# robotics-upo/social_force_window_planner

Measured on AMD Instinct MI355X. Metric: scored trajectories/sec (v x w samples x steps) @ N pedestrians; cmd_vel match, higher is better.
Workload: dtype f64

## Files before the change

include/sfw_hip.h:

```cpp
#ifndef SFW_HIP_H_
#define SFW_HIP_H_

#include <stdint.h>

#ifdef __cplusplus
extern "C" {
#endif

#define SFW_ABI_VERSION 2

typedef enum sfw_status {
  SFW_OK = 0,
  SFW_ERR_INVALID_ARG = -1,
  SFW_ERR_NO_DEVICE = -2,
  SFW_ERR_HIP = -3,
  SFW_ERR_STATE = -4,
  SFW_ERR_UNSUPPORTED = -5
} sfw_status;

#define SFW_COST_INVALID (-1.0)
#define SFW_COST_SKIPPED (-2.0)

#define SFW_ROBOT_ID_NONE INT32_MIN

// ... 155 lines not shown
int sfw_plan_shared_prefix(const double *linvels, int32_t nv,
                           const double *angvels, int32_t nw, double vx0,
                           double vtheta0, double acc_x, double acc_theta,
                           double sim_time, int32_t num_steps,
                           int32_t n_agents, int32_t *level_ends,
                           int64_t *level_classes, int32_t cap,
                           int32_t *n_levels);
int sfw_plan_axis_classes(const double *targets, int32_t n, double v0, double a_max, double dt, int32_t max_p,
                          int32_t form, int32_t *counts, int32_t *classes, int32_t *n_levels, int32_t *closed_form);
int sfw_plan_row_blocks(const double *linvels, int32_t nv, const double *angvels, int32_t nw, double vx0,
                        double vtheta0, double acc_x, double acc_theta, double sim_time, int32_t num_steps,
                        int32_t n_agents, int32_t R, int32_t *row0);
#define SFW_K2_AUTO (-1)
#define SFW_K2_REGISTER 0
#define SFW_K2_FLAT 1
int sfw_set_k2_form(sfw_handle h, int32_t form);
int sfw_set_timing(sfw_handle h, int32_t enabled);
int sfw_last_launch_ms(sfw_handle h, int32_t which, float *ms_out);
int sfw_last_clock_ghz(sfw_handle h, double *ghz_out);
int sfw_grid_points(sfw_handle h, int64_t index, double *points_xyth,
                    int32_t points_cap, int32_t *n_points);
int sfw_grid_points_batch(sfw_handle h, int64_t first, int64_t count, double *points_xyth, int32_t *n_points);
int sfw_set_points_capture(sfw_handle h, int32_t enabled);
void *sfw_stream(sfw_handle h);

#define SFW_TERM_VEL 0
#define SFW_TERM_DISTANCE 1
#define SFW_TERM_ANGLE 2
#define SFW_TERM_COSTMAP 3
#define SFW_TERM_SOCIAL 4
#define SFW_N_TERMS 5
#define SFW_RESCORE_MAX_K 1024
typedef struct sfw_weights {
  double vel, distance, angle, costmap, social;
} sfw_weights;
int sfw_set_terms_capture(sfw_handle h, int32_t enabled);
int sfw_grid_rescore(sfw_handle h, const sfw_weights *w, int32_t K, sfw_best *best_out, double *costs_out);
int sfw_grid_terms(sfw_handle h, int64_t first, int64_t count, double *terms_out);

#define SFW_BLEND_MAX_L 16
typedef struct sfw_blend_stat {
  double lambda;
  double j_min;
  double eta;
  double sum_w2;
  int64_t n_valid;
// ... 135 lines not shown
```

social_force_window_planner_amd/_abi.py:

```python
import ctypes as C

SFW_OK = 0
SFW_ERR_INVALID_ARG = -1
SFW_ERR_NO_DEVICE = -2
SFW_ERR_HIP = -3
SFW_ERR_STATE = -4
SFW_ERR_UNSUPPORTED = -5

SFW_COST_INVALID = -1.0
SFW_COST_SKIPPED = -2.0

SFW_PRECISION_F64 = 0
SFW_PRECISION_F32 = 1
SFW_PRECISION_F64_STRICT = 2

SFW_K2_AUTO, SFW_K2_REGISTER, SFW_K2_FLAT = -1, 0, 1
SFW_ORG_NONE, SFW_ORG_REGISTER_1, SFW_ORG_REGISTER_2, SFW_ORG_FLAT = 0, 1, 2, 3


class SfwParams(C.Structure):
    _fields_ = [
        ("max_vel_x", C.c_double),
        ("sim_time", C.c_double),
        ("sim_granularity", C.c_double),
# ... 190 lines not shown
    "sfw_ensemble_aggregate",
    "sfw_ensemble_last_us",
    "sfw_samples_stage",
    "sfw_score_samples",
    "sfw_sequences_stage",
    "sfw_score_sequences",
    "sfw_score_one_crowd",
    "sfw_grid_crowd",
    "sfw_grid_blend",
    "sfw_sequences_perturb_stage",
    "sfw_score_perturbed",
    "sfw_sequences_knots",
    "sfw_sequences_normals",
    "sfw_ensemble_score_sequences",
    "sfw_ensemble_score_perturbed",
    "sfw_ensemble_blend",
    "sfw_sequences_control_cost",
    "sfw_grid_blend_control",
    "sfw_mppi_run",
    "sfw_ensemble_blend_control",
    "sfw_ensemble_mppi_run",
    "sfw_ensemble_set_risk",
    "sfw_ensemble_get_risk",
)
SFW_TERM_VEL, SFW_TERM_DISTANCE, SFW_TERM_ANGLE, SFW_TERM_COSTMAP, SFW_TERM_SOCIAL = 0, 1, 2, 3, 4
SFW_N_TERMS = 5
SFW_RESCORE_MAX_K = 1024


class SfwWeights(C.Structure):

    _fields_ = [("vel", C.c_double), ("distance", C.c_double), ("angle", C.c_double), ("costmap", C.c_double),
                ("social", C.c_double)]


SFW_BLEND_MAX_L = 16


class SfwBlendStat(C.Structure):

    _fields_ = [("lambda_", C.c_double), ("j_min", C.c_double), ("eta", C.c_double), ("sum_w2", C.c_double),
                ("n_valid", C.c_int64), ("index_min", C.c_int64)]

    def as_dict(self):
        d = {"lambda": self.lambda_, "j_min": self.j_min, "eta": self.eta, "sum_w2": self.sum_w2, "n_valid": self.n_valid,
             "index_min": self.index_min}
# ... 71 lines not shown
```

social_force_window_planner_amd/csrc/sfw_capi.hip:

```cpp

#include "sfw_device.h"

#include <dlfcn.h>
#include <link.h>

#include <algorithm>
#include <chrono>
#include <cmath>
#include <condition_variable>
#include <functional>
#include <mutex>
#include <thread>
#include <cstdio>
#include <cstdlib>
#include <cstring>
#include <limits>
#include <new>
#include <string>
#include <vector>

namespace {

template <typename T> struct dev_buf {
  T *p = nullptr;
  size_t cap = 0;
  dev_buf() = default;
  dev_buf(const dev_buf &) = delete;
  dev_buf &operator=(const dev_buf &) = delete;
  hipError_t reserve(size_t n) {
    if (n <= cap) return hipSuccess;
    if (p) (void)hipFree(p);
    p = nullptr;
    cap = 0;
    size_t want = n + n / 8 + 16;
    hipError_t e = hipMalloc(reinterpret_cast<void **>(&p), want * sizeof(T));
    if (e == hipSuccess) cap = want;
    return e;
  }
  void release() {
    if (p) (void)hipFree(p);
    p = nullptr;
    cap = 0;
  }
};

struct pinned_buf {
  char *p = nullptr;
  size_t cap = 0;
  hipEvent_t done = nullptr;
  bool pending = false;
  pinned_buf() = default;
  pinned_buf(const pinned_buf &) = delete;
  pinned_buf &operator=(const pinned_buf &) = delete;
  hipError_t wait() {
    if (!pending) return hipSuccess;
    pending = false;
    return hipEventSynchronize(done);
  }
  hipError_t reserve(size_t bytes) {
    hipError_t e = wait();
    if (e != hipSuccess) return e;
    if (!done && (e = hipEventCreateWithFlags(&done, hipEventDisableTiming)) != hipSuccess) return e;
    if (bytes <= cap) return hipSuccess;
    if (p) (void)hipHostFree(p);
    p = nullptr;
    cap = 0;
    const size_t want = bytes + bytes / 4 + 256;
    e = hipHostMalloc(reinterpret_cast<void **>(&p), want, hipHostMallocDefault);
// ... 53 lines not shown
  dev_buf<double> ctrl_bias, mppi_plan;
  pinned_buf pin_mppi;
  void release() {
    ctrl_bias.release();
    mppi_plan.release();
    pin_mppi.release();
  }
};

}

struct sfw_planner_s {
  struct config {
    int n_cu = SFW_DEFAULT_CUS, n_xcd = SFW_DEFAULT_CUS / SFW_CUS_PER_XCD;
    std::vector<int> prefix_env;
    bool pin_rest_on = true;
    long spin_us = 20000;
    bool arena_direct_on = true;
    size_t mirror_max_bytes = size_t(64) << 20;
    int obs_tasks_force = -1;
    size_t table_budget_bytes = size_t(8) << 30;
    bool owns_streams = true;
    bool batch_member = false;
  } cfg;

  struct switches {
    sfw_params params;
    uint64_t params_epoch = 1;
    int k2_form = SFW_K2_AUTO;
    bool timing = false;
    bool capture_points = false;
    bool capture_terms = false;
  } live;

  struct world_state {
    map_geometry map_new{0, 0, 0, 0, 0};
    bool have_costmap = false;
    bool cells_dirty = false;
    std::vector<double> footprint;
    int K = 0;
    agent_set agents;
  } world;

  struct stage_record {
    bool valid = false;
    std::vector<double> lin, ang;
    int nv = 0, nw = 0;
    sfw_robot_state rs{};
    sfw_goal_args ga{};
    double vy_samp = 0.0;
    int skip_zero = 1;
    int64_t index_base = 0;
    bool list = false;
    std::vector<double> vy;
    int nk = 1;
    std::vector<int32_t> knot_step;
    const int32_t *d_knot_step = nullptr;
    bool perturbed = false, zero_admitted = false, normals_kept = false;
    sfw_perturb_dev pert{};
    int K = 0, A = 0, O = 0, NG = 0, n_grp_mem = 0;
    bool person_pinned = false;
// ... 12 lines not shown
    std::vector<std::pair<int32_t, int32_t>> rest_pairs;
    std::vector<double> rest_pv;
    size_t pin_doubles = 0;
    std::vector<double> pin_pos;
    std::vector<sfw_agent_const> pin_cst;
    std::vector<int> prefix_steps;
    std::vector<chunk_plan> prefix_chunks;
    size_t prefix_o_col_cls = 0;
    int prefix_S = 0;
    int64_t prefix_chunk = 0;
    int64_t prefix_class_steps = 0, prefix_last_classes = 0;
    std::vector<int32_t> cls_ints;
    int64_t cls_max = 0;
    bool cls_two = false;
    const int32_t *d_cls_tab = nullptr;
    int64_t table_chunk = 0;
    uint64_t plan_epoch = 0;
    bool arena_pending = false;
    size_t arena_from = 0, arena_bytes = 0;
    bool early_poses = false;
    bool early_poses_timed = false;
    bool early_poses_terms = false;
    bool clock_cleared = false;
  } st;

  struct launch_record {
    bool launched = false;
    bool timed = false;
    bool cycle = false;
    bool fetched = false;
    bool mirrored = false;
    bool captured = false;
    int cap_S = 0;
    bool terms = false;
    int n_chunks = 1;
  } last;
  uint64_t launch_seq = 0;

  int device = 0;
  hipStream_t stream = nullptr;
  hipStream_t side = nullptr;
  hipEvent_t ev_poses = nullptr, ev_side = nullptr;
  sfw_split_streams split{nullptr, nullptr, nullptr};
  hipEvent_t ev[5] = {nullptr, nullptr, nullptr, nullptr, nullptr};
  std::vector<hipEvent_t> chunk_ev;
  std::string err;
  const void *shared_cols = nullptr;

  dev_buf<uint8_t> cells;
  dev_buf<char> arena;
  dev_buf<uint16_t> pair_tab;
  int pair_tab_A = -1;
  dev_buf<unsigned> cycle_counter;
  dev_buf<int32_t> d_cls, cls_dead[2];
  dev_buf<sfw_cls_agent> cls_state[2];
  dev_buf<int32_t> status, coll_step;
  dev_buf<double> base_cost, costs;
  dev_buf<sfw_unit> ptab, cs_tab;
  dev_buf<int16_t> fcode;
  dev_buf<sfw_sel> partials;
  dev_buf<double> points;
  dev_buf<int32_t> n_points;
  dev_buf<unsigned long long> clock;
  dev_buf<char> one_out;
  dev_buf<int32_t> pts_status, pts_coll;
  dev_buf<double> pts_base, pts_costs;
  dev_buf<sfw_unit> pts_ptab, pts_cs;
  dev_buf<int16_t> pts_fcode;
  pinned_buf pin_map, pin_arena, pin_out, pin_cls;
  pinned_buf pin_one;
  pinned_buf pin_mirror;
  pinned_buf pin_cap;
  dev_buf<double> terms;
  dev_buf<sfw_weights> rescore_w;
  dev_buf<sfw_sel> rescore_partials;
  dev_buf<double> rescore_costs;
  pinned_buf pin_rescore;
  blend_buffers blend;
  mppi_buffers mppi;
  dev_buf<double> normals;
  pinned_buf pin_knots;
  dev_buf<char> crowd_out;
// ... 106 lines not shown
  L.rs = h->st.rs;
  L.ga = h->st.ga;
  L.vy_samp = h->st.vy_samp;
  L.skip_zero_sample = h->st.skip_zero;
  L.linvels = h->st.d_linvels;
  L.angvels = h->st.d_angvels;
  L.nv = h->st.nv;
  L.nw = h->st.nw;
  L.vy_samps = h->st.d_vy;
  L.list = h->st.list ? 1 : 0;
  L.n_knots = h->st.nk;
  L.knot_step = h->st.d_knot_step;
  L.knot_stride = h->st.nv;
  L.chunk_begin = begin;
  L.chunk_count = count;
  L.cells = h->st.d_cells;
  L.size_x = h->st.map.size_x;
  L.size_y = h->st.map.size_y;
  L.origin_x = h->st.map.origin_x;
  L.origin_y = h->st.map.origin_y;
  L.resolution = h->st.map.resolution;
  L.footprint = h->st.d_footprint;
  L.K = h->st.K;
  L.agent_pos = h->st.d_agent_pos;
  L.agent_vel = h->st.d_agent_vel;
  L.agent_c = h->st.d_agent_c;
  L.agent_rest = h->st.d_agent_rest;
  L.pin_rest = h->st.d_pin_rest;
  L.A = h->st.A;
  L.obstacles = h->st.d_obstacles;
  L.O = h->st.O;
  L.agent_grp = h->st.d_agent_grp;
  L.grp_off = h->st.d_grp_off;
  L.grp_mem = h->st.d_grp_mem;
  L.NG = h->st.NG;
  L.n_grp_mem = h->st.n_grp_mem;
  L.n_cu = h->cfg.n_cu;
  L.n_xcd = h->cfg.n_xcd;
  sfw_derive(L);
  if (h->cfg.obs_tasks_force >= 0 && L.O > 0) L.k.obs_tasks = h->cfg.obs_tasks_force;
  L.pair_tab = h->pair_tab.p;
  L.status = h->status.p;
  L.base_cost = h->base_cost.p;
  L.costs = h->costs.p;
  L.coll_step = h->coll_step.p;
  L.ptab = h->ptab.p;
// ... 668 lines not shown
  return {stage_request::LIST, vx, vy, vtheta, n, 1, 1, nullptr, nullptr, 0.0, 0, index_base};
}
stage_request sequences_request(const double *vx, const double *vy, const double *vtheta, int32_t n, int32_t K,
                                const int32_t *knot_step, int64_t index_base) {
  return {stage_request::SEQUENCES, vx, vy, vtheta, n, 1, K, knot_step, nullptr, 0.0, 0, index_base};
}
stage_request perturbed_request(const perturb_source *dev, int32_t n, int32_t K, const int32_t *knot_step, int64_t index_base) {
  return {stage_request::PERTURBED, nullptr, nullptr, nullptr, n, 1, K, knot_step, dev, 0.0, 0, index_base};
}

const char *stage_null_refusal(const sfw_robot_state *rs, const sfw_goal_args *args, const stage_request &q) {
  if (!rs || (!q.drawn() && (!q.lin || !q.ang)) || !args || q.nv <= 0 || q.nw <= 0) return "null pointer or non-positive sample count";
  return nullptr;
}
const char *stage_finite_refusal(const sfw_robot_state *rs, const sfw_goal_args *args, const stage_request &q) {
  if (!all_finite(&rs->x, 6) || !all_finite(&args->acc_x, 5) || !std::isfinite(q.vy_samp))
    return "non-finite robot state, goal argument or sample velocity";
  const size_t rows = q.kn() * static_cast<size_t>(q.nv);
  if (!q.drawn() && (!all_finite(q.lin, rows) || !all_finite(q.ang, q.kn() * q.n_ang()) || (q.vy_list && !all_finite(q.vy_list, rows))))
    return "non-finite sample velocity";
  return nullptr;
}

int stage_common(sfw_handle h, const sfw_robot_state *rs, const sfw_goal_args *args, const stage_request &q) {
  if (!h) return SFW_ERR_INVALID_ARG;
  const std::string what = q.name();
  const auto [kind, lin, vy_list, ang, nv, nw, nk, knot_step, dev, vy_samp, skip_zero, index_base] = q;
  const size_t kn = q.kn(), n_ang = q.n_ang();
  const bool has_vy = dev ? dev->vy : vy_list != nullptr;
  if (const char *why = stage_null_refusal(rs, args, q)) return fail(h, SFW_ERR_INVALID_ARG, what + ": " + why);
  if (!h->world.have_costmap) return fail(h, SFW_ERR_STATE, what + ": no costmap set (sfw_set_costmap)");
  if (const char *why = stage_finite_refusal(rs, args, q)) return fail(h, SFW_ERR_INVALID_ARG, what + ": " + why);
  drop_stage(h);
  host_phases ph("stage:");
  SFW_HIP(h, hipSetDevice(h->device));
  const agent_set &ag = h->world.agents;
  const map_geometry &map = h->world.map_new;
  const size_t n_cells = static_cast<size_t>(map.size_x) * map.size_y;
  const bool merge = n_cells <= kMapMergeMax;
  if (h->world.cells_dirty && !merge) {
    SFW_HIP(h, h->cells.reserve(n_cells));
    SFW_HIP(h, hipMemcpyAsync(h->cells.p, h->pin_map.p, n_cells, hipMemcpyHostToDevice, h->stream));
    SFW_HIP(h, h->pin_map.mark(h->stream));
    h->world.cells_dirty = false;
  }
  ph.mark("check+setdev");
  h->st.perturbed = dev != nullptr;
  h->st.zero_admitted = dev && dev->zero_admitted;
  if (dev) h->st.pert = dev->args;
  h->st.normals_kept = false;
  if (dev) {
    h->st.lin.clear();
    h->st.ang.clear();
  } else {
    h->st.lin.assign(lin, lin + kn * nv);
    h->st.ang.assign(ang, ang + kn * n_ang);
  }
  h->st.list = q.is_list();
  if (vy_list) h->st.vy.assign(vy_list, vy_list + kn * nv);
  else h->st.vy.clear();
  h->st.nk = static_cast<int>(kn);
  if (knot_step) h->st.knot_step.assign(knot_step, knot_step + kn);
  else h->st.knot_step.clear();
  h->st.K = h->world.K;
  h->st.A = ag.A;
  h->st.O = ag.O;
  h->st.NG = ag.NG;
  h->st.n_grp_mem = ag.n_grp_mem;
  h->st.person_pinned = ag.person_pinned;
  h->st.nv = nv;
  h->st.nw = nw;
  h->st.rs = *rs;
  h->st.ga = *args;
  h->st.vy_samp = vy_samp;
  h->st.skip_zero = skip_zero;
  h->st.index_base = index_base;
  h->st.map = map;
  int plan_err = SFW_OK;
  const int64_t chunk = plan_tables_host(h, &plan_err);
  if (plan_err) return plan_err;
  ph.mark("plan");
  auto up16 = [](size_t b) { return (b + 15) & ~size_t(15); };
  const size_t cells_head = merge ? up16(n_cells) : 0;
  {
    const bool rest = !ag.rest_pairs.empty();
    const size_t o_fp = cells_head, o_ag = o_fp + up16(sizeof(double) * (h->world.footprint.empty() ? 2 : h->world.footprint.size())),
                 o_lin = o_ag + up16(ag.blob.size()), o_ang = o_lin + up16(sizeof(double) * kn * nv),
// ... 82 lines not shown
  const int64_t T = static_cast<int64_t>(nv) * nw;
  SFW_HIP(h, h->status.reserve(T));
  SFW_HIP(h, h->coll_step.reserve(T));
  SFW_HIP(h, h->base_cost.reserve(T));
  SFW_HIP(h, h->costs.reserve(T + (sizeof(sfw_sel) + sizeof(double) - 1) / sizeof(double)));
  h->st.d_sel = reinterpret_cast<sfw_sel *>(h->costs.p + T);
  SFW_HIP(h, h->partials.reserve(sfw_argmin_partials(T)));
  ph.mark("reserve");
  if (dev) {
    double *z = nullptr;
    if (dev->keep_normals) {
      SFW_HIP(h, h->normals.reserve(3 * kn * static_cast<size_t>(nv)));
      z = h->normals.p;
    }
    SFW_HIP(h, sfw_launch_perturb(dev->args, nv, static_cast<int>(kn), index_base, const_cast<double *>(h->st.d_linvels),
                                  const_cast<double *>(h->st.d_vy), const_cast<double *>(h->st.d_angvels), z, h->stream));
    h->st.normals_kept = dev->keep_normals;
    ph.mark("perturb");
  }
  if (int e = plan_tables_device(h, chunk, true)) return e;
  if (T > 1024)
    if (int e = flush_arena(h)) return e;
  ph.mark("tables+K1a");
  if (merge) {
    h->world.cells_dirty = false;
    h->st.cells_in_arena = true;
    h->st.arena_cells_bytes = cells_head;
  }
  h->st.valid = true;
  return SFW_OK;
}

int flush_arena(sfw_handle h) {
  if (!h->st.arena_pending) return SFW_OK;
  h->st.arena_pending = false;
  hipError_t e = hipMemcpyAsync(h->arena.p + h->st.arena_from, h->pin_arena.p + h->st.arena_from, h->st.arena_bytes,
                                hipMemcpyHostToDevice, h->stream);
  if (e == hipSuccess) e = h->pin_arena.mark(h->stream);
  if (e != hipSuccess) {
    drop_stage(h);
    return hip_fail(h, e, "flush_arena: arena copy");
  }
  return SFW_OK;
}

struct launch_prep {
// ... 591 lines not shown
  if (hipGetDeviceCount(&count) != hipSuccess || count <= 0) return SFW_ERR_NO_DEVICE;
  if (device < 0 || device >= count) return SFW_ERR_INVALID_ARG;
  sfw_handle h = new (std::nothrow) sfw_planner_s();
  if (!h) return SFW_ERR_HIP;
  h->live.params = *params;
  h->device = device;
  if (const char *b = std::getenv("SFW_PREFIX")) {
    for (const char *q = b; *q;) {
      char *end = nullptr;
      const long v = std::strtol(q, &end, 10);
      if (end == q) break;
      if (v >= 0) h->cfg.prefix_env.push_back(static_cast<int>(v));
      q = (*end == ',') ? end + 1 : end;
    }
    std::sort(h->cfg.prefix_env.begin(), h->cfg.prefix_env.end());
    h->cfg.prefix_env.erase(std::unique(h->cfg.prefix_env.begin(), h->cfg.prefix_env.end()), h->cfg.prefix_env.end());
  }
  if (const char *b = std::getenv("SFW_FORCE_FLAT")) h->live.k2_form = std::atoi(b) == 1 ? SFW_K2_FLAT : std::atoi(b) == 0 ? SFW_K2_REGISTER : SFW_K2_AUTO;
  if (const char *b = std::getenv("SFW_PIN_REST")) h->cfg.pin_rest_on = std::atoi(b) != 0;
  if (const char *b = std::getenv("SFW_SPIN_US")) h->cfg.spin_us = std::max(0L, std::atol(b));
  if (const char *b = std::getenv("SFW_ARENA_DIRECT")) h->cfg.arena_direct_on = std::atoi(b) != 0;
  if (const char *b = std::getenv("SFW_MIRROR_MAX_MB")) h->cfg.mirror_max_bytes = static_cast<size_t>(std::max(0L, std::atol(b))) << 20;
  if (const char *b = std::getenv("SFW_OBS_TASKS")) h->cfg.obs_tasks_force = std::atoi(b) != 0 ? 1 : 0;
  if (const char *b = std::getenv("SFW_TABLE_BUDGET_MB")) {
    long mb = std::atol(b);
    if (mb > 0) h->cfg.table_budget_bytes = static_cast<size_t>(mb) << 20;
  }
  hipError_t e = hipSetDevice(device);
  if (e == hipSuccess) {
    hipDeviceProp_t prop;
    if (hipGetDeviceProperties(&prop, device) == hipSuccess && prop.multiProcessorCount > 0) h->cfg.n_cu = prop.multiProcessorCount;
    h->cfg.n_cu = env_device_cus(h->cfg.n_cu);
    int xccs = 0;
    if (!std::getenv("SFW_DEVICE_CUS") && hipDeviceGetAttribute(&xccs, hipDeviceAttributeNumberOfXccs, device) == hipSuccess && xccs >= 1)
      h->cfg.n_xcd = xccs;
    else
      h->cfg.n_xcd = std::max(1, h->cfg.n_cu / SFW_CUS_PER_XCD);
    (void)hipGetLastError();
    if (const char *b = std::getenv("SFW_DEVICE_XCDS")) {
      const long v = std::atol(b);
      if (v >= 1 && v <= 64) h->cfg.n_xcd = static_cast<int>(v);
    }
  }
  if (stream) {
    h->cfg.owns_streams = false;
    h->stream = stream;
// ... 15 lines not shown
    return SFW_ERR_HIP;
  }
  *out = h;
  return SFW_OK;
}

int destroy_handle(sfw_handle h) {
  (void)hipSetDevice(h->device);
  if (h->stream) (void)hipStreamSynchronize(h->stream);
  if (h->side) (void)hipStreamSynchronize(h->side);
  h->cells.release();
  h->arena.release();
  h->pair_tab.release();
  h->crowd_pair_tab.release();
  h->crowd_out.release();
  h->pin_crowd.release();
  h->status.release();
  h->coll_step.release();
  h->base_cost.release();
  h->costs.release();
  h->ptab.release();
  h->cs_tab.release();
  h->fcode.release();
  h->partials.release();
  h->clock.release();
  h->cycle_counter.release();
  h->pin_cap.release();
  h->terms.release();
  h->rescore_w.release();
  h->rescore_partials.release();
  h->rescore_costs.release();
  h->pin_rescore.release();
  h->blend.release();
  h->mppi.release();
  h->normals.release();
  h->pin_knots.release();
  h->points.release();
  h->n_points.release();
  h->one_out.release();
  h->pts_status.release();
  h->pts_coll.release();
  h->pts_base.release();
  h->pts_costs.release();
  h->pts_ptab.release();
  h->pts_cs.release();
  h->pts_fcode.release();
// ... 44 lines not shown
}

const char *sfw_last_error(sfw_handle h) { return h ? h->err.c_str() : "null handle"; }

int sfw_set_costmap(sfw_handle h, const uint8_t *cells, uint32_t size_x, uint32_t size_y, double origin_x,
                    double origin_y, double resolution) {
  if (!h) return SFW_ERR_INVALID_ARG;
  if (!cells || size_x == 0 || size_y == 0 || !(resolution > 0))
    return fail(h, SFW_ERR_INVALID_ARG, "set_costmap: null cells, zero size or non-positive resolution");
  if (!std::isfinite(origin_x) || !std::isfinite(origin_y) || !std::isfinite(resolution))
    return fail(h, SFW_ERR_INVALID_ARG, "set_costmap: origin or resolution is not finite");
  if (size_x > SFW_MAX_MAP_AXIS_CELLS || size_y > SFW_MAX_MAP_AXIS_CELLS || static_cast<uint64_t>(size_x) * size_y > SFW_MAX_MAP_CELLS)
    return fail(h, SFW_ERR_INVALID_ARG, "set_costmap: more than SFW_MAX_MAP_AXIS_CELLS cells on an axis or SFW_MAX_MAP_CELLS in all");
  SFW_HIP(h, hipSetDevice(h->device));
  const size_t n = static_cast<size_t>(size_x) * size_y;
  if (h->world.have_costmap && h->pin_map.p && n <= h->pin_map.cap && h->world.map_new.size_x == size_x && h->world.map_new.size_y == size_y &&
      h->world.map_new.origin_x == origin_x && h->world.map_new.origin_y == origin_y && h->world.map_new.resolution == resolution &&
      std::memcmp(h->pin_map.p, cells, n) == 0)
    return SFW_OK;
  SFW_HIP(h, h->pin_map.reserve(n));
  std::memcpy(h->pin_map.p, cells, n);
  h->world.map_new = {size_x, size_y, origin_x, origin_y, resolution};
  h->world.cells_dirty = true;
  h->world.have_costmap = true;
  return SFW_OK;
}

int sfw_set_footprint(sfw_handle h, const double *xy, int32_t K) {
  if (!h) return SFW_ERR_INVALID_ARG;
  if (K < 0 || (K > 0 && !xy)) return fail(h, SFW_ERR_INVALID_ARG, "set_footprint: bad arguments");
  h->world.footprint.assign(xy, xy + 2 * static_cast<size_t>(K));
  h->world.K = K;
  return SFW_OK;
}

int sfw_set_agents(sfw_handle h, const sfw_agent *agents, int32_t A, const double *obstacles_xy, int32_t O) {
  if (!h) return SFW_ERR_INVALID_ARG;
  if (A < 0 || O < 0 || (A > 0 && !agents) || (O > 0 && !obstacles_xy))
    return fail(h, SFW_ERR_INVALID_ARG, "set_agents: bad arguments");
  for (int i = 0; i < A; ++i) {
    const sfw_agent &a = agents[i];
    if (!all_finite(&a.x, 4) || !std::isfinite(a.desired_velocity) || !std::isfinite(a.radius) ||
        (a.has_goal && !(all_finite(&a.goal_x, 2) && std::isfinite(a.goal_radius))))
      return fail(h, SFW_ERR_INVALID_ARG, "set_agents: non-finite field in agent " + std::to_string(i));
  }
  if (O > 0 && !all_finite(obstacles_xy, 2 * static_cast<size_t>(O)))
// ... 362 lines not shown
      float ms = 0.0f;
      const int a = 3 * c + (which == 1 ? 0 : 1);
      SFW_HIP(h, hipEventElapsedTime(&ms, h->chunk_ev[a], h->chunk_ev[a + 1]));
      total += ms;
    }
    *ms_out = total;
    return SFW_OK;
  }
  int a = 0, b = 3;
  switch (which) {
    case 0: a = 0; b = 3; break;
    case 1: a = 0; b = 1; break;
    case 2: a = 1; b = 2; break;
    case 3: a = 2; b = 3; break;
    default: return fail(h, SFW_ERR_INVALID_ARG, "last_launch_ms: which must be 0..3");
  }
  SFW_HIP(h, hipEventElapsedTime(ms_out, h->ev[a], h->ev[b]));
  return SFW_OK;
}

int sfw_set_points_capture(sfw_handle h, int32_t enabled) {
  if (!h) return SFW_ERR_INVALID_ARG;
  h->live.capture_points = enabled != 0;
  return SFW_OK;
}

int sfw_set_terms_capture(sfw_handle h, int32_t enabled) {
  if (!h) return SFW_ERR_INVALID_ARG;
  h->live.capture_terms = enabled != 0;
  if (!h->live.capture_terms) {
    h->last.terms = false;
    h->st.early_poses_terms = false;
    if (h->terms.p) {
      SFW_HIP(h, hipSetDevice(h->device));
      SFW_HIP(h, hipStreamSynchronize(h->stream));
      h->terms.release();
    }
  }
  return SFW_OK;
}

int sfw_grid_rescore(sfw_handle h, const sfw_weights *w, int32_t K, sfw_best *best_out, double *costs_out) {
  if (!h) return SFW_ERR_INVALID_ARG;
  if (!w || !best_out) return fail(h, SFW_ERR_INVALID_ARG, "grid_rescore: weights or best_out is NULL");
  if (K < 1 || K > SFW_RESCORE_MAX_K) return fail(h, SFW_ERR_INVALID_ARG, "grid_rescore: K out of [1, SFW_RESCORE_MAX_K]");
  if (!all_finite(reinterpret_cast<const double *>(w), static_cast<size_t>(K) * SFW_N_TERMS))
// ... 1614 lines not shown
```

social_force_window_planner_amd/csrc/sfw_device.h:

```cpp
#ifndef SFW_DEVICE_H_
#define SFW_DEVICE_H_

#include <hip/hip_runtime.h>
#include <stdint.h>

#include "../../include/sfw_hip.h"


#define SFW_DEFAULT_CUS 256
#define SFW_CUS_PER_XCD 32

enum : int32_t { SFW_ST_VALID = 0, SFW_ST_INVALID = 1, SFW_ST_SKIPPED = 2 };

struct __attribute__((aligned(32))) sfw_robot_step {
  double x, y, vx, vy;
};

struct __attribute__((aligned(32))) sfw_pose_frame {
  double x, y, c, s;
};

struct __attribute__((aligned(16))) sfw_unit {
  double a, b;
};
// ... 100 lines not shown
  sfw_unit *ptab;
  sfw_unit *cs_tab;
  int64_t row_units;
  int16_t *fcode;
  int64_t rstep_stride;
  double *points;
  int32_t *n_points;
  unsigned long long *clock_probe;
  int64_t index_base;
  unsigned *cycle_counter;
  sfw_sel *sel_out;
  double *costs_host;
  sfw_sel *sel_host;
  const char *arena_host;
  char *arena_dev;
  uint32_t arena_bytes;
  double *terms;
  int64_t terms_T;
  const double *vy_samps;
  int32_t list;
  int32_t n_knots;
  const int32_t *knot_step;
  int64_t knot_stride;
};

__device__ __forceinline__ void sfw_put_term(double *terms, int64_t T, int64_t t, int k, double v) {
  if (terms) terms[k * T + t] = v;
}
__device__ __forceinline__ void sfw_put_terms3(double *terms, int64_t T, int64_t t, double vel, double d, double ang) {
  if (!terms) return;
  terms[SFW_TERM_VEL * T + t] = vel;
  terms[SFW_TERM_DISTANCE * T + t] = d;
  terms[SFW_TERM_ANGLE * T + t] = ang;
}
__device__ __forceinline__ void sfw_put_terms_sentinel(double *terms, int64_t T, int64_t t, double sentinel) {
  if (!terms) return;
  for (int k = 0; k < SFW_N_TERMS; ++k) terms[k * T + t] = sentinel;
}


struct sfw_crowd_out {
  double *state;
  double *work;
  int32_t *has_goal;
};

void sfw_derive(sfw_launch &L);

hipError_t sfw_launch_rollout(const sfw_launch &L, hipStream_t stream);
hipError_t sfw_launch_rollout_poses(const sfw_launch &L, hipStream_t stream);
hipError_t sfw_launch_rollout_costmap(const sfw_launch &L, hipStream_t stream);
struct sfw_split_streams {
  hipStream_t side;
  hipEvent_t fork, join;
};
hipError_t sfw_launch_social(const sfw_launch &L, hipStream_t stream, const sfw_split_streams *sp = nullptr);
bool sfw_cycle_applies(const sfw_launch &L);
hipError_t sfw_launch_cycle(const sfw_launch &L, hipStream_t stream);
#define SFW_BATCH_VARIANTS 27
struct sfw_batch_rec {
  sfw_launch L;
  int32_t k2_bytes;
  int32_t lds_bytes;
};
inline size_t sfw_batch_recs_offset(int B) { return (sizeof(uint32_t) * (static_cast<size_t>(B) + 1) + 15) & ~size_t(15); }
int sfw_cycle_batch_variant(const sfw_launch &L);
void sfw_cycle_batch_record(const sfw_launch &L, sfw_batch_rec *rec);
hipError_t sfw_launch_cycle_batch(int variant, const uint32_t *d_first, const sfw_batch_rec *d_recs, int B, unsigned blocks,
                                  size_t lds, hipStream_t stream);
#ifndef SFW_STRICT_BUILD
hipError_t sfw_launch_cycle_batch_strict(int variant, const uint32_t *d_first, const sfw_batch_rec *d_recs, int B,
                                         unsigned blocks, size_t lds, hipStream_t stream);
int64_t sfw_social_flat_items(int A, int O, int NG, int64_t T, int form, int cus);
hipError_t sfw_launch_social_strict(const sfw_launch &L, hipStream_t stream, const sfw_split_streams *sp = nullptr);
// ... 73 lines not shown
```

social_force_window_planner_amd/csrc/sfw_kernels.hip:

```cpp

#include "sfw_device.h"
#include "sfw_math.h"

#include <type_traits>

#include <limits.h>
#include <math.h>
#include <stdlib.h>
#include <cmath>

namespace {

constexpr int WAVE = 64;

#pragma clang fp contract(off)

__device__ __forceinline__ unsigned cell_index(double a, double res, double inv_res) {
  const double q = a * inv_res;
  const double m = __builtin_trunc(q);
  const double d = q - m;
  if (d < 1e-9 || d > 1.0 - 1e-9) return static_cast<unsigned>(a / res);
  return static_cast<unsigned>(m);
}

// ... 10 lines not shown
}

__device__ __forceinline__ int line_max(const sfw_launch &L, int x0, int y0, int x1, int y1) {
  const int dx = x1 - x0, dy = y1 - y0;
  const int adx = abs(dx), ady = abs(dy);
  const int stride = static_cast<int>(L.size_x);
  const int sx = (dx >= 0) ? 1 : -1, sy = (dy >= 0) ? stride : -stride;
  const bool x_major = adx >= ady;
  const int den = x_major ? adx : ady, add = x_major ? ady : adx;
  const int dmaj = x_major ? sx : sy, dmin = x_major ? sy : sx;
  int num = den / 2;
  unsigned idx = static_cast<unsigned>(y0 * stride + x0);
  int best = 0;
  for (int n = 0; n <= den; ++n) {
    best = max(best, static_cast<int>(L.cells[idx]));
    num += add;
    const bool wrap = num >= den;
    num -= wrap ? den : 0;
    idx += static_cast<unsigned>(dmaj + (wrap ? dmin : 0));
  }
  return best;
}

__device__ double footprint_cost(const sfw_launch &L, double x, double y, double c, double s) {
  const double inv_res = 1.0 / L.resolution;
  unsigned cx, cy;
  if (!world_to_map(L, inv_res, x, y, cx, cy)) return -3.0;
  const int K = L.K;
  if (K < 3) {
    const int code = point_code(L, (int)cx, (int)cy);
    if (code == 255) return -2.0;
    if (code == 254 || code == 253) return -1.0;
    return static_cast<double>(code);
  }
  int fc = 0;
  double qx = L.footprint[0], qy = L.footprint[1];
  unsigned fx0, fy0;
  if (!world_to_map(L, inv_res, x + (qx * c - qy * s), y + (qx * s + qy * c), fx0, fy0)) return -3.0;
  unsigned x0 = fx0, y0 = fy0;
  for (int e = 0; e < K; ++e) {
    unsigned x1, y1;
    if (e + 1 < K) {
      qx = L.footprint[2 * (e + 1)];
      qy = L.footprint[2 * (e + 1) + 1];
      if (!world_to_map(L, inv_res, x + (qx * c - qy * s), y + (qx * s + qy * c), x1, y1)) return -3.0;
    } else {
      x1 = fx0;
      y1 = fy0;
    }
    fc = max(fc, line_max(L, (int)x0, (int)y0, (int)x1, (int)y1));
    x0 = x1;
    y0 = y1;
  }
  return static_cast<double>(fc);
}

__device__ __forceinline__ double new_velocity(double vg, double vi, double a_max, double dt) {
  const double step = a_max * dt;
  const double up = fmin(vg, vi + step), dn = fmax(vg, vi - step);
  return (vg - vi) >= 0 ? up : dn;
}
__device__ __forceinline__ float normalize_angle_f(float val, float mn, float mx) {
  if (val >= mn) return mn + fmodf(val - mn, mx - mn);
  return mx - fmodf(mn - val, mx - mn);
}

__device__ __forceinline__ int64_t vel_row_of(const sfw_launch &L, int64_t local) {
  return (L.chunk_begin + local) / L.nw - L.chunk_begin / L.nw;
}
template <bool LIST>
__device__ __forceinline__ void put_robot_step(const sfw_launch &L, int64_t local, int i, double xn, double yn, double vx,
                                               double vy, double c, double s) {
  sfw_unit *const row = L.ptab + static_cast<int64_t>(i) * L.row_units;
  row[local] = sfw_unit{xn, yn};
  if constexpr (LIST) {
    row[L.rstep_stride + local] = sfw_unit{vx, vy};
    L.cs_tab[static_cast<int64_t>(i) * L.rstep_stride + local] = sfw_unit{c, s};
// ... 229 lines not shown
        double *pt = L.points + (local * S + i) * 3;
        pt[0] = r_px[g][j];
        pt[1] = r_py[g][j];
        pt[2] = thq;
      }
      put_robot_step<LIST>(L, local, i, r_px[g][j + 1], r_py[g][j + 1], vxq, vyq, c, s);
    }
  }
  if (j < 3) r_end[g][j] = j == 2 ? th_i : p;
  if (j == 0) r_end[g][3] = v;
  __syncthreads();
  if (j == 0 && live) {
    const double dx = L.ga.wpx - r_end[g][0], dy = L.ga.wpy - r_end[g][1];
    const double d = dx * dx + dy * dy;
    double ang = atan2(dy, dx) - r_end[g][2];
    ang = normalize_angle_f(static_cast<float>(ang), static_cast<float>(-M_PI), static_cast<float>(M_PI));
    ang = fabs(ang) / M_PI;
    const double vel = fabs(L.p.max_vel_x - r_end[g][3]) / L.p.max_vel_x;
    L.base_cost[t] = sfw_cost_base(L.p.vel_weight, vel, L.p.distance_weight, d, L.p.angle_weight, ang);
    if (scored) sfw_put_terms3(L.terms, L.terms_T, t, vel, d, ang);
  }
}

template <bool LIST> __global__ void __launch_bounds__(256) sfw_footprint_kernel(const sfw_launch L) {
  const int64_t idx = static_cast<int64_t>(blockIdx.x) * blockDim.x + threadIdx.x;
  const int64_t n = L.chunk_count;
  if (idx >= n * L.S) return;
  const int64_t step = idx / n, local = idx - step * n;
  if (L.status[L.chunk_begin + local] == SFW_ST_SKIPPED) return;
  const sfw_unit pos = step == 0 ? sfw_unit{L.rs.x, L.rs.y} : L.ptab[(step - 1) * L.row_units + local];
  const sfw_unit cs = LIST ? L.cs_tab[step * L.rstep_stride + local] : L.cs_tab[step * L.nw + (L.chunk_begin + local) % L.nw];
  const double fc = footprint_cost(L, pos.a, pos.b, cs.a, cs.b);
  L.fcode[step * L.rstep_stride + local] = static_cast<int16_t>(fc);
}

__global__ void __launch_bounds__(256) sfw_costmap_scan_kernel(const sfw_launch L) {
  const int64_t local = static_cast<int64_t>(blockIdx.x) * blockDim.x + threadIdx.x;
  if (local >= L.chunk_count) return;
  const int64_t t = L.chunk_begin + local;
  if (L.status[t] == SFW_ST_SKIPPED) {
    if (L.n_points) L.n_points[local] = 0;
    return;
  }
  const int S = L.S;
  double cm = 0.0;
  int n_ok = 0;
  bool stopped = false;
  for (int base = 0; base < S && !stopped; base += 8) {
    int16_t v[8];
#pragma unroll
    for (int j = 0; j < 8; ++j)
      v[j] = (base + j < S) ? L.fcode[static_cast<int64_t>(base + j) * L.rstep_stride + local] : int16_t(-1);
#pragma unroll
    for (int j = 0; j < 8; ++j)
      if (!stopped && base + j < S) stopped = !scan_code(static_cast<double>(v[j]), cm, n_ok);
  }
  scan_finish(L, t, local, cm, n_ok);
// ... 2570 lines not shown
  if (sfw_rollout_is_fused(L)) {
    hipLaunchKernelGGL((L.n_knots > 1 ? sfw_rollout_small_kernel<true, true> : L.list ? sfw_rollout_small_kernel<true> : sfw_rollout_small_kernel<false>),
                       dim3(static_cast<unsigned>(L.chunk_count)), dim3(K1_SMALL_BLOCK), 0, stream, L);
    return hipGetLastError();
  }
  const int block = 64;
  if (sfw_k1a_threads()) {
    const unsigned grid = static_cast<unsigned>((L.chunk_count + block - 1) / block);
    hipLaunchKernelGGL((L.n_knots > 1 ? sfw_rollout_kernel<true, true> : L.list ? sfw_rollout_kernel<true> : sfw_rollout_kernel<false>),
                       dim3(grid), dim3(block), 0, stream, L);
    return hipGetLastError();
  }
  constexpr int per_wave = WAVE / K1A_TEAM;
  const unsigned grid = static_cast<unsigned>((L.chunk_count + per_wave - 1) / per_wave);
  hipLaunchKernelGGL((L.n_knots > 1 ? sfw_rollout_team_kernel<true, true> : L.list ? sfw_rollout_team_kernel<true> : sfw_rollout_team_kernel<false>),
                     dim3(grid), dim3(block), 0, stream, L);
  return hipGetLastError();
}

hipError_t sfw_launch_rollout_costmap(const sfw_launch &L, hipStream_t stream) {
  if (L.chunk_count <= 0 || sfw_rollout_is_fused(L)) return hipSuccess;
  {
    const int block = 256;
    const int64_t n = L.chunk_count * L.S;
    const unsigned grid = static_cast<unsigned>((n + block - 1) / block);
    hipLaunchKernelGGL((L.list ? sfw_footprint_kernel<true> : sfw_footprint_kernel<false>), dim3(grid), dim3(block), 0, stream, L);
  }
  {
    const int block = 256;
    const unsigned grid = static_cast<unsigned>((L.chunk_count + block - 1) / block);
    hipLaunchKernelGGL(sfw_costmap_scan_kernel, dim3(grid), dim3(block), 0, stream, L);
  }
  return hipGetLastError();
}

hipError_t sfw_launch_rollout(const sfw_launch &L, hipStream_t stream) {
  hipError_t e = sfw_launch_rollout_poses(L, stream);
  return e != hipSuccess ? e : sfw_launch_rollout_costmap(L, stream);
}

template <typename K> static hipError_t launch_social_as(K kernel, const sfw_launch &L, int G, unsigned grid,
                                                          size_t lds, hipStream_t stream) {
  if (lds > 64 * 1024) {
    hipError_t e = hipFuncSetAttribute(reinterpret_cast<const void *>(kernel),
                                       hipFuncAttributeMaxDynamicSharedMemorySize, static_cast<int>(lds));
    if (e != hipSuccess) return e;
  }
  hipLaunchKernelGGL(kernel, dim3(grid), dim3(WAVE), lds, stream, L, G);
  return hipGetLastError();
}

template <int CAP> static bool reg_layout_matches() {
  const lds_layout s(nullptr, 5, CAP, 10, 2, 3, 0, 0, true, false);
  auto at = [&](const void *p) { return static_cast<int>(reinterpret_cast<const char *>(p) - reinterpret_cast<const char *>(s.px)); };
  using off = reg_off<CAP>;
  return at(s.py) == off::PY && at(s.vx) == off::VX && at(s.vy) == off::VY && at(s.fjx) == off::FJX && at(s.fjy) == off::FJY &&
         at(s.hasgoal) == off::HG && at(s.swp) == off::SW && at(s.dead) == off::DEAD && at(s.rsb) == off::RSB && s.hg_stride == 2;
// ... 442 lines not shown
```

social_force_window_planner_amd/planner.py:

```python
from __future__ import annotations

import ctypes as C
import os
import subprocess

import numpy as np

from ._abi import (
    EXPORTED_SYMBOLS,
    SFW_ENSEMBLE_MAX,
    SFW_ENSEMBLE_MEAN,
    SFW_ERR_NO_DEVICE,
    SFW_OK,
    SfwAgent,
    SfwBatchDesc,
    SfwBest,
    SfwBestKey,
    SfwBlendStat,
    SFW_BLEND_MAX_L,
    SfwGoalArgs,
    SfwMppi,
    SFW_MPPI_MAX_ITER,
    SfwParams,
    SfwPerturb,
# ... 145 lines not shown
        L.sfw_ensemble_score_sequences.argtypes = [vp, C.POINTER(SfwRobotState), vp, vp, vp, C.c_int32, C.c_int32, vp,
                                                   C.POINTER(SfwGoalArgs), C.c_int32, vp, vp, vp, C.POINTER(SfwBest)]
        L.sfw_ensemble_score_perturbed.argtypes = [vp, C.POINTER(SfwRobotState), C.POINTER(SfwPerturb), C.c_int32, C.c_int32, vp,
                                                   C.POINTER(SfwGoalArgs), C.c_int32, vp, vp, vp, C.POINTER(SfwBest)]
        L.sfw_ensemble_blend.argtypes = [vp, vp, C.c_int32, vp, C.POINTER(SfwBlendStat), vp, vp]
        L.sfw_sequences_control_cost.argtypes = [vp, C.c_double, vp]
        L.sfw_grid_blend_control.argtypes = [vp, vp, C.c_int32, C.c_double, vp, C.POINTER(SfwBlendStat), vp, vp]
        L.sfw_mppi_run.argtypes = [vp, C.POINTER(SfwRobotState), C.POINTER(SfwPerturb), C.c_int32, C.c_int32, vp,
                                   C.POINTER(SfwGoalArgs), C.POINTER(SfwMppi), C.POINTER(SfwBlendStat), vp, C.POINTER(SfwBest)]
        L.sfw_ensemble_blend_control.argtypes = [vp, vp, C.c_int32, C.c_double, vp, C.POINTER(SfwBlendStat), vp, vp]
        L.sfw_ensemble_mppi_run.argtypes = [vp, C.POINTER(SfwRobotState), C.POINTER(SfwPerturb), C.c_int32, C.c_int32, vp,
                                            C.POINTER(SfwGoalArgs), C.c_int32, vp, C.POINTER(SfwMppi), C.POINTER(SfwBlendStat), vp,
                                            vp, vp, C.POINTER(SfwBest)]
        L.sfw_ensemble_set_risk.argtypes = [vp, C.POINTER(SfwRisk)]
        L.sfw_ensemble_get_risk.argtypes = [vp, C.POINTER(SfwRisk), C.POINTER(C.c_int32)]
        L.sfw_batch_set_list_fusion.argtypes = [vp, C.c_int32]
        L.sfw_batch_get_list_fusion.argtypes = [vp, C.POINTER(C.c_int32)]
        L.sfw_batch_score_samples.argtypes = [vp, vp, vp, vp, vp, C.c_int32, vp, vp]
        L.sfw_batch_score_sequences.argtypes = [vp, vp, vp, vp, vp, C.c_int32, C.c_int32, vp, vp, vp]
        L.sfw_batch_score_perturbed.argtypes = [vp, vp, vp, C.c_int32, C.c_int32, vp, vp, vp]
        L.sfw_ensemble_set_list_fusion.argtypes = [vp, C.c_int32]
        L.sfw_ensemble_get_list_fusion.argtypes = [vp, C.POINTER(C.c_int32)]
        L.sfw_ensemble_batch_desc.argtypes = [vp, C.POINTER(SfwBatchDesc), C.POINTER(C.c_int64)]
        _lib = L
    return _lib


def exported_symbols():
    L = lib()
    return {name: hasattr(L, name) for name in EXPORTED_SYMBOLS}


def _f64(a):
    return np.ascontiguousarray(a, dtype=np.float64)


class _Owner:
    _members = ()

    def close(self):
        if getattr(self, self._attr, None):
            for m in self._members:
                m.close()
            getattr(lib(), self._destroy)(getattr(self, self._attr))
            setattr(self, self._attr, C.c_void_p())

# ... 276 lines not shown
    def plan_info(self):
        info = SfwPlanInfo()
        self._check(lib().sfw_grid_plan_info(self._h, C.byref(info)), "sfw_grid_plan_info")
        return info.as_dict()

    def set_k2_form(self, form):
        self._check(lib().sfw_set_k2_form(self._h, form), "sfw_set_k2_form")

    def set_timing(self, enabled=True):
        self._check(lib().sfw_set_timing(self._h, 1 if enabled else 0), "sfw_set_timing")

    def last_launch_ms(self, which=0):
        ms = C.c_float()
        self._check(lib().sfw_last_launch_ms(self._h, which, C.byref(ms)), "sfw_last_launch_ms")
        return ms.value

    def sustained_clock_ghz(self):
        v = C.c_double()
        self._check(lib().sfw_last_clock_ghz(self._h, C.byref(v)), "sfw_last_clock_ghz")
        return v.value

    def set_points_capture(self, enabled=True):
        self._check(lib().sfw_set_points_capture(self._h, 1 if enabled else 0), "sfw_set_points_capture")

    def grid_points_batch(self, first, count, n_steps):
        pts = np.zeros((count, n_steps, 3), dtype=np.float64)
        n = np.zeros(count, dtype=np.int32)
        self._check(lib().sfw_grid_points_batch(self._h, first, count, pts.ctypes.data, n.ctypes.data),
                    "sfw_grid_points_batch")
        return pts, n

    def grid_points(self, index, points_cap=4096):
        pts = np.zeros((points_cap, 3), dtype=np.float64)
        n = C.c_int32()
        self._check(lib().sfw_grid_points(self._h, index, pts.ctypes.data, points_cap, C.byref(n)),
                    "sfw_grid_points")
        return pts[: min(n.value, points_cap)].copy()

    def _num_steps(self):
        n = int(self.params.sim_time / self.params.sim_granularity + 0.5)
        return n if n != 0 else 1

    @staticmethod
    def _crowd_buffers(cap, A):
        n = max(cap, 1) * max(A, 1)
        return (np.zeros(4 * n, dtype=np.float64)[: 4 * max(cap, 1) * A].reshape(max(cap, 1), A, 4),
# ... 547 lines not shown
```

Measured before the change: 7.771 million.

## Skip footprint cost via precomputed clearance map of obstacle-free neighborhoods

```diff
diff --git a/include/sfw_hip.h b/include/sfw_hip.h
--- a/include/sfw_hip.h
+++ b/include/sfw_hip.h
@@ -201,6 +201,9 @@
                     int32_t points_cap, int32_t *n_points);
 int sfw_grid_points_batch(sfw_handle h, int64_t first, int64_t count, double *points_xyth, int32_t *n_points);
 int sfw_set_points_capture(sfw_handle h, int32_t enabled);
+int sfw_set_footprint_clearance(sfw_handle h, int32_t on);
+int sfw_footprint_clearance_info(sfw_handle h, int32_t *built, int32_t *half_width);
+int sfw_footprint_clearance_map(sfw_handle h, uint8_t *out, uint64_t cells);
 void *sfw_stream(sfw_handle h);
 
 #define SFW_TERM_VEL 0
diff --git a/social_force_window_planner_amd/_abi.py b/social_force_window_planner_amd/_abi.py
--- a/social_force_window_planner_amd/_abi.py
+++ b/social_force_window_planner_amd/_abi.py
@@ -236,6 +236,9 @@
     "sfw_ensemble_mppi_run",
     "sfw_ensemble_set_risk",
     "sfw_ensemble_get_risk",
+    "sfw_set_footprint_clearance",
+    "sfw_footprint_clearance_info",
+    "sfw_footprint_clearance_map",
 )
 SFW_TERM_VEL, SFW_TERM_DISTANCE, SFW_TERM_ANGLE, SFW_TERM_COSTMAP, SFW_TERM_SOCIAL = 0, 1, 2, 3, 4
 SFW_N_TERMS = 5
diff --git a/social_force_window_planner_amd/csrc/sfw_capi.hip b/social_force_window_planner_amd/csrc/sfw_capi.hip
--- a/social_force_window_planner_amd/csrc/sfw_capi.hip
+++ b/social_force_window_planner_amd/csrc/sfw_capi.hip
@@ -44,6 +44,9 @@
   }
 };
 
+constexpr int kClearMaxHalfWidth = 64;
+constexpr int64_t kClearMinPoses = 368640;
+
 struct pinned_buf {
   char *p = nullptr;
   size_t cap = 0;
@@ -143,6 +146,7 @@
     size_t table_budget_bytes = size_t(8) << 30;
     bool owns_streams = true;
     bool batch_member = false;
+    int64_t clear_min_poses = kClearMinPoses;
   } cfg;
 
   struct switches {
@@ -152,12 +156,14 @@
     bool timing = false;
     bool capture_points = false;
     bool capture_terms = false;
+    bool fp_clear = true;
   } live;
 
   struct world_state {
     map_geometry map_new{0, 0, 0, 0, 0};
     bool have_costmap = false;
     bool cells_dirty = false;
+    uint64_t cells_gen = 0;
     std::vector<double> footprint;
     int K = 0;
     agent_set agents;
@@ -216,7 +222,16 @@
     bool early_poses_timed = false;
     bool early_poses_terms = false;
     bool clock_cleared = false;
+    bool clear_on = false;
+    int clear_r = -1;
   } st;
+
+  struct clearance_record {
+    bool valid = false;
+    uint64_t cells_gen = 0;
+    uint32_t size_x = 0, size_y = 0;
+    int r = 0;
+  } clr;
 
   struct launch_record {
     bool launched = false;
@@ -252,6 +267,7 @@
   dev_buf<double> base_cost, costs;
   dev_buf<sfw_unit> ptab, cs_tab;
   dev_buf<int16_t> fcode;
+  dev_buf<uint8_t> clear_map, clear_tmp;
   dev_buf<sfw_sel> partials;
   dev_buf<double> points;
   dev_buf<int32_t> n_points;
@@ -404,6 +420,7 @@
   L.resolution = h->st.map.resolution;
   L.footprint = h->st.d_footprint;
   L.K = h->st.K;
+  L.clear = (h->live.fp_clear && h->st.clear_on) ? h->clear_map.p : nullptr;
   L.agent_pos = h->st.d_agent_pos;
   L.agent_vel = h->st.d_agent_vel;
   L.agent_c = h->st.d_agent_c;
@@ -1118,6 +1135,40 @@
   return nullptr;
 }
 
+int clearance_half_width(const std::vector<double> &footprint, double resolution) {
+  double R = 0.0;
+  for (size_t i = 0; i + 1 < footprint.size(); i += 2) R = std::fmax(R, std::hypot(footprint[i], footprint[i + 1]));
+  const double q = std::ceil(R / resolution) + 1.0;
+  return q <= kClearMaxHalfWidth ? static_cast<int>(q) : -1;
+}
+
+void stage_clearance(sfw_handle h, int64_t T) {
+  h->st.clear_on = false;
+  h->st.clear_r = -1;
+  if (!h->live.fp_clear) return;
+  const map_geometry &m = h->st.map;
+  const int r = clearance_half_width(h->world.footprint, m.resolution);
+  h->st.clear_r = r;
+  if (r < 0) return;
+  auto &c = h->clr;
+  if (c.valid && c.cells_gen == h->world.cells_gen && c.size_x == m.size_x && c.size_y == m.size_y && c.r == r) {
+    h->st.clear_on = true;
+    return;
+  }
+  if (T * num_steps_of(h->live.params) < h->cfg.clear_min_poses) return;
+  c.valid = false;
+  const size_t n = static_cast<size_t>(m.size_x) * m.size_y;
+  hipError_t e = h->clear_map.reserve(n);
+  if (e == hipSuccess) e = h->clear_tmp.reserve(n);
+  if (e == hipSuccess) e = sfw_launch_clearance(h->st.d_cells, m.size_x, m.size_y, r, h->clear_tmp.p, h->clear_map.p, h->stream);
+  if (e != hipSuccess) {
+    (void)hipGetLastError();
+    return;
+  }
+  c = {true, h->world.cells_gen, m.size_x, m.size_y, r};
+  h->st.clear_on = true;
+}
+
 int stage_common(sfw_handle h, const sfw_robot_state *rs, const sfw_goal_args *args, const stage_request &q) {
   if (!h) return SFW_ERR_INVALID_ARG;
   const std::string what = q.name();
@@ -1159,6 +1210,7 @@
   if (knot_step) h->st.knot_step.assign(knot_step, knot_step + kn);
   else h->st.knot_step.clear();
   h->st.K = h->world.K;
+  h->st.clear_on = false;
   h->st.A = ag.A;
   h->st.O = ag.O;
   h->st.NG = ag.NG;
@@ -1287,6 +1339,8 @@
   if (T > 1024)
     if (int e = flush_arena(h)) return e;
   ph.mark("tables+K1a");
+  stage_clearance(h, T);
+  ph.mark("clearance");
   if (merge) {
     h->world.cells_dirty = false;
     h->st.cells_in_arena = true;
@@ -1924,6 +1978,7 @@
   if (const char *b = std::getenv("SFW_ARENA_DIRECT")) h->cfg.arena_direct_on = std::atoi(b) != 0;
   if (const char *b = std::getenv("SFW_MIRROR_MAX_MB")) h->cfg.mirror_max_bytes = static_cast<size_t>(std::max(0L, std::atol(b))) << 20;
   if (const char *b = std::getenv("SFW_OBS_TASKS")) h->cfg.obs_tasks_force = std::atoi(b) != 0 ? 1 : 0;
+  if (const char *b = std::getenv("SFW_CLEAR_MIN_POSES")) h->cfg.clear_min_poses = std::max(0LL, std::atoll(b));
   if (const char *b = std::getenv("SFW_TABLE_BUDGET_MB")) {
     long mb = std::atol(b);
     if (mb > 0) h->cfg.table_budget_bytes = static_cast<size_t>(mb) << 20;
@@ -1985,6 +2040,8 @@
   h->ptab.release();
   h->cs_tab.release();
   h->fcode.release();
+  h->clear_map.release();
+  h->clear_tmp.release();
   h->partials.release();
   h->clock.release();
   h->cycle_counter.release();
@@ -2075,6 +2132,7 @@
   std::memcpy(h->pin_map.p, cells, n);
   h->world.map_new = {size_x, size_y, origin_x, origin_y, resolution};
   h->world.cells_dirty = true;
+  ++h->world.cells_gen;
   h->world.have_costmap = true;
   return SFW_OK;
 }
@@ -2483,6 +2541,32 @@
 int sfw_set_points_capture(sfw_handle h, int32_t enabled) {
   if (!h) return SFW_ERR_INVALID_ARG;
   h->live.capture_points = enabled != 0;
+  return SFW_OK;
+}
+
+int sfw_set_footprint_clearance(sfw_handle h, int32_t on) {
+  if (!h) return SFW_ERR_INVALID_ARG;
+  h->live.fp_clear = on != 0;
+  return SFW_OK;
+}
+
+int sfw_footprint_clearance_info(sfw_handle h, int32_t *built, int32_t *half_width) {
+  if (!h) return SFW_ERR_INVALID_ARG;
+  if (!built || !half_width) return fail(h, SFW_ERR_INVALID_ARG, "footprint_clearance_info: null pointer");
+  if (!h->st.valid) return fail(h, SFW_ERR_STATE, "footprint_clearance_info: nothing is staged");
+  *built = (h->live.fp_clear && h->st.clear_on) ? 1 : 0;
+  *half_width = h->st.clear_r;
+  return SFW_OK;
+}
+
+int sfw_footprint_clearance_map(sfw_handle h, uint8_t *out, uint64_t cells) {
+  if (!h) return SFW_ERR_INVALID_ARG;
+  if (!h->st.valid || !h->st.clear_on) return fail(h, SFW_ERR_STATE, "footprint_clearance_map: the staged grid has no clearance map");
+  if (!out || cells != static_cast<uint64_t>(h->st.map.size_x) * h->st.map.size_y)
+    return fail(h, SFW_ERR_INVALID_ARG, "footprint_clearance_map: null buffer, or not size_x * size_y cells");
+  SFW_HIP(h, hipSetDevice(h->device));
+  SFW_HIP(h, hipMemcpyAsync(out, h->clear_map.p, cells, hipMemcpyDeviceToHost, h->stream));
+  SFW_HIP(h, hipStreamSynchronize(h->stream));
   return SFW_OK;
 }
 
diff --git a/social_force_window_planner_amd/csrc/sfw_device.h b/social_force_window_planner_amd/csrc/sfw_device.h
--- a/social_force_window_planner_amd/csrc/sfw_device.h
+++ b/social_force_window_planner_amd/csrc/sfw_device.h
@@ -146,6 +146,7 @@
   int32_t n_knots;
   const int32_t *knot_step;
   int64_t knot_stride;
+  const uint8_t *clear;
 };
 
 __device__ __forceinline__ void sfw_put_term(double *terms, int64_t T, int64_t t, int k, double v) {
@@ -174,6 +175,8 @@
 hipError_t sfw_launch_rollout(const sfw_launch &L, hipStream_t stream);
 hipError_t sfw_launch_rollout_poses(const sfw_launch &L, hipStream_t stream);
 hipError_t sfw_launch_rollout_costmap(const sfw_launch &L, hipStream_t stream);
+hipError_t sfw_launch_clearance(const uint8_t *cells, uint32_t size_x, uint32_t size_y, int r, uint8_t *tmp, uint8_t *clear,
+                                hipStream_t stream);
 struct sfw_split_streams {
   hipStream_t side;
   hipEvent_t fork, join;
diff --git a/social_force_window_planner_amd/csrc/sfw_kernels.hip b/social_force_window_planner_amd/csrc/sfw_kernels.hip
--- a/social_force_window_planner_amd/csrc/sfw_kernels.hip
+++ b/social_force_window_planner_amd/csrc/sfw_kernels.hip
@@ -56,10 +56,8 @@
   return best;
 }
 
-__device__ double footprint_cost(const sfw_launch &L, double x, double y, double c, double s) {
-  const double inv_res = 1.0 / L.resolution;
-  unsigned cx, cy;
-  if (!world_to_map(L, inv_res, x, y, cx, cy)) return -3.0;
+__device__ double footprint_cost_at(const sfw_launch &L, double inv_res, unsigned cx, unsigned cy, double x, double y, double c,
+                                    double s) {
   const int K = L.K;
   if (K < 3) {
     const int code = point_code(L, (int)cx, (int)cy);
@@ -87,6 +85,19 @@
     y0 = y1;
   }
   return static_cast<double>(fc);
+}
+__device__ double footprint_cost(const sfw_launch &L, double x, double y, double c, double s) {
+  const double inv_res = 1.0 / L.resolution;
+  unsigned cx, cy;
+  if (!world_to_map(L, inv_res, x, y, cx, cy)) return -3.0;
+  return footprint_cost_at(L, inv_res, cx, cy, x, y, c, s);
+}
+__device__ double footprint_cost_clear(const sfw_launch &L, double x, double y, double c, double s) {
+  const double inv_res = 1.0 / L.resolution;
+  unsigned cx, cy;
+  if (!world_to_map(L, inv_res, x, y, cx, cy)) return -3.0;
+  if (L.clear && L.clear[static_cast<size_t>(cy) * L.size_x + cx]) return 0.0;
+  return footprint_cost_at(L, inv_res, cx, cy, x, y, c, s);
 }
 
 __device__ __forceinline__ double new_velocity(double vg, double vi, double a_max, double dt) {
@@ -362,17 +373,36 @@
   }
 }
 
-template <bool LIST> __global__ void __launch_bounds__(256) sfw_footprint_kernel(const sfw_launch L) {
-  const int64_t idx = static_cast<int64_t>(blockIdx.x) * blockDim.x + threadIdx.x;
-  const int64_t n = L.chunk_count;
-  if (idx >= n * L.S) return;
-  const int64_t step = idx / n, local = idx - step * n;
+template <bool LIST> __global__ void __launch_bounds__(256) sfw_footprint_kernel(const sfw_launch L, const int step0) {
+  const int64_t local = static_cast<int64_t>(blockIdx.x) * blockDim.x + threadIdx.x;
+  if (local >= L.chunk_count) return;
+  const int64_t step = static_cast<int64_t>(step0) + blockIdx.y;
   if (L.status[L.chunk_begin + local] == SFW_ST_SKIPPED) return;
   const sfw_unit pos = step == 0 ? sfw_unit{L.rs.x, L.rs.y} : L.ptab[(step - 1) * L.row_units + local];
   const sfw_unit cs = LIST ? L.cs_tab[step * L.rstep_stride + local] : L.cs_tab[step * L.nw + (L.chunk_begin + local) % L.nw];
-  const double fc = footprint_cost(L, pos.a, pos.b, cs.a, cs.b);
+  const double fc = footprint_cost_clear(L, pos.a, pos.b, cs.a, cs.b);
   L.fcode[step * L.rstep_stride + local] = static_cast<int16_t>(fc);
 }
+
+#ifndef SFW_STRICT_BUILD
+__global__ void __launch_bounds__(256) sfw_clearance_rows_kernel(const uint8_t *cells, int size_x, int size_y, int y0, int r, uint8_t *tmp) {
+  const int x = blockIdx.x * blockDim.x + threadIdx.x, y = y0 + blockIdx.y;
+  if (x >= size_x || y >= size_y) return;
+  const uint8_t *row = cells + static_cast<size_t>(y) * size_x;
+  int m = (x - r < 0 || x + r >= size_x) ? 255 : 0;
+  const int lo = max(x - r, 0), hi = min(x + r, size_x - 1);
+  for (int i = lo; i <= hi; ++i) m = max(m, static_cast<int>(row[i]));
+  tmp[static_cast<size_t>(y) * size_x + x] = static_cast<uint8_t>(m);
+}
+__global__ void __launch_bounds__(256) sfw_clearance_cols_kernel(const uint8_t *tmp, int size_x, int size_y, int y0, int r, uint8_t *clear) {
+  const int x = blockIdx.x * blockDim.x + threadIdx.x, y = y0 + blockIdx.y;
+  if (x >= size_x || y >= size_y) return;
+  int m = (y - r < 0 || y + r >= size_y) ? 255 : 0;
+  const int lo = max(y - r, 0), hi = min(y + r, size_y - 1);
+  for (int j = lo; j <= hi; ++j) m = max(m, static_cast<int>(tmp[static_cast<size_t>(j) * size_x + x]));
+  clear[static_cast<size_t>(y) * size_x + x] = m == 0 ? 1 : 0;
+}
+#endif
 
 __global__ void __launch_bounds__(256) sfw_costmap_scan_kernel(const sfw_launch L) {
   const int64_t local = static_cast<int64_t>(blockIdx.x) * blockDim.x + threadIdx.x;
@@ -2989,9 +3019,11 @@
   if (L.chunk_count <= 0 || sfw_rollout_is_fused(L)) return hipSuccess;
   {
     const int block = 256;
-    const int64_t n = L.chunk_count * L.S;
-    const unsigned grid = static_cast<unsigned>((n + block - 1) / block);
-    hipLaunchKernelGGL((L.list ? sfw_footprint_kernel<true> : sfw_footprint_kernel<false>), dim3(grid), dim3(block), 0, stream, L);
+    const unsigned grid = static_cast<unsigned>((L.chunk_count + block - 1) / block);
+    for (int step0 = 0; step0 < L.S; step0 += 65535) {
+      const unsigned steps = static_cast<unsigned>(L.S - step0 < 65535 ? L.S - step0 : 65535);
+      hipLaunchKernelGGL((L.list ? sfw_footprint_kernel<true> : sfw_footprint_kernel<false>), dim3(grid, steps), dim3(block), 0, stream, L, step0);
+    }
   }
   {
     const int block = 256;
@@ -3000,6 +3032,25 @@
   }
   return hipGetLastError();
 }
+
+#ifndef SFW_STRICT_BUILD
+hipError_t sfw_launch_clearance(const uint8_t *cells, uint32_t size_x, uint32_t size_y, int r, uint8_t *tmp, uint8_t *clear,
+                                hipStream_t stream) {
+  const int block = 256;
+  const unsigned gx = (size_x + block - 1) / block;
+  for (int pass = 0; pass < 2; ++pass)
+    for (uint32_t y0 = 0; y0 < size_y; y0 += 65535u) {
+      const uint32_t ny = (size_y - y0 < 65535u) ? size_y - y0 : 65535u;
+      if (pass == 0)
+        hipLaunchKernelGGL(sfw_clearance_rows_kernel, dim3(gx, ny), dim3(block), 0, stream, cells, static_cast<int>(size_x),
+                           static_cast<int>(size_y), static_cast<int>(y0), r, tmp);
+      else
+        hipLaunchKernelGGL(sfw_clearance_cols_kernel, dim3(gx, ny), dim3(block), 0, stream, tmp, static_cast<int>(size_x),
+                           static_cast<int>(size_y), static_cast<int>(y0), r, clear);
+    }
+  return hipGetLastError();
+}
+#endif
 
 hipError_t sfw_launch_rollout(const sfw_launch &L, hipStream_t stream) {
   hipError_t e = sfw_launch_rollout_poses(L, stream);
diff --git a/social_force_window_planner_amd/planner.py b/social_force_window_planner_amd/planner.py
--- a/social_force_window_planner_amd/planner.py
+++ b/social_force_window_planner_amd/planner.py
@@ -191,6 +191,9 @@
         L.sfw_ensemble_set_list_fusion.argtypes = [vp, C.c_int32]
         L.sfw_ensemble_get_list_fusion.argtypes = [vp, C.POINTER(C.c_int32)]
         L.sfw_ensemble_batch_desc.argtypes = [vp, C.POINTER(SfwBatchDesc), C.POINTER(C.c_int64)]
+        L.sfw_set_footprint_clearance.argtypes = [vp, C.c_int32]
+        L.sfw_footprint_clearance_info.argtypes = [vp, C.POINTER(C.c_int32), C.POINTER(C.c_int32)]
+        L.sfw_footprint_clearance_map.argtypes = [vp, vp, C.c_uint64]
         _lib = L
     return _lib
 
@@ -513,6 +516,19 @@
 
     def set_points_capture(self, enabled=True):
         self._check(lib().sfw_set_points_capture(self._h, 1 if enabled else 0), "sfw_set_points_capture")
+
+    def set_footprint_clearance(self, enabled=True):
+        self._check(lib().sfw_set_footprint_clearance(self._h, 1 if enabled else 0), "sfw_set_footprint_clearance")
+
+    def footprint_clearance_info(self):
+        built, r = C.c_int32(), C.c_int32()
+        self._check(lib().sfw_footprint_clearance_info(self._h, C.byref(built), C.byref(r)), "sfw_footprint_clearance_info")
+        return bool(built.value), r.value
+
+    def footprint_clearance_map(self, size_y, size_x):
+        out = np.zeros((size_y, size_x), dtype=np.uint8)
+        self._check(lib().sfw_footprint_clearance_map(self._h, out.ctypes.data, out.size), "sfw_footprint_clearance_map")
+        return out
 
     def grid_points_batch(self, first, count, n_steps):
         pts = np.zeros((count, n_steps, 3), dtype=np.float64)
```

New measurement: 7.867 million (median of 6 runs). 1.01x the previous value.
